# MTG/DeepConvSep

Hardware: NVIDIA H100
Metric: audio_seconds_separated_per_second (higher is better)
Workload: dtype f32

## Files before the change

### deepconvsep_b200/csrc/api.cu

```cuda
#include <stdarg.h>
#include <math.h>
#include <string.h>
#include <stdlib.h>
#include <map>
#include <mutex>
#include <utility>
#include <vector>
#include "common.cuh"

namespace dcs {

static thread_local char g_err[1024] = "";

void set_error(const char* fmt, ...) {
  va_list ap;
  va_start(ap, fmt);
  vsnprintf(g_err, sizeof(g_err), fmt, ap);
  va_end(ap);
}

int DevBuf::ensure(size_t bytes, cudaStream_t stream, bool* grew) {
  if (grew) *grew = false;
  if (bytes <= cap) return DCS_OK;
  if (p) {
// ... 330 lines not shown
}

static bool score_arch(int arch) { return arch == DCS_ARCH_BACH10_SCORE || arch == DCS_ARCH_BACH10_SCORE_1X1; }
static int score_planes(const dcs_model* m) { return m->arch == DCS_ARCH_BACH10_SCORE_1X1 ? 4 : m->sc.nch; }

static int check_model(const char* fn, const dcs_ctx* ctx, const dcs_model* m, int arch, int overlap, int patcher) {
  DCS_REQUIRE(ctx && m, "%s: NULL argument", fn);
  const bool mono = m->arch != DCS_ARCH_DSD_ILD && !score_arch(m->arch);
  DCS_REQUIRE(arch < 0 ? mono : (arch == DCS_ARCH_BACH10_SCORE ? score_arch(m->arch) : m->arch == arch),
              "%s does not serve architecture %d: use %s", fn, m->arch,
              m->arch == DCS_ARCH_DSD_ILD ? "dcs_separate_audio_stereo"
              : score_arch(m->arch)       ? "dcs_separate_audio_score / dcs_separate_spec_channels"
                                          : "dcs_separate_audio / dcs_separate_spec");
  DCS_REQUIRE(overlap >= 0 && overlap < m->tc, "overlap %d must be in [0, time_context=%d)", overlap, m->tc);
  DCS_REQUIRE(patcher == DCS_PATCHER_STANDALONE || patcher == DCS_PATCHER_UTIL, "unknown patcher %d", patcher);
  return DCS_OK;
}

static int check_clip(const char* fn, const dcs_ctx* ctx, const dcs_model* m, const dcs_stft* p, int arch, const void* in,
                      const void* out, int64_t L, int64_t in_stride, int64_t out_stride, int overlap, int patcher) {
  DCS_TRY(check_model(fn, ctx, m, arch, overlap, patcher));
  DCS_REQUIRE(p && in && out, "%s: NULL argument", fn);
  DCS_REQUIRE(p->N / 2 + 1 == m->F, "%s: frame size %d does not give the model's %d bins", fn, p->N, m->F);
  DCS_REQUIRE(L > 0 && in_stride >= L && out_stride >= L, "%s: bad length / stride", fn);
  return DCS_OK;
}

static int size_workspace(dcs_ctx* ctx, const dcs_model* m, const dcs_stft* p, int64_t L, bool staged, cudaStream_t st,
                          bool masks = false) {
  const int64_t plane = dcs_num_frames(L, p->hop) * dcs_padded_bins(p->N);
  if (!masks) DCS_TRY(ctx->X.ensure((size_t)m->nch * plane * sizeof(float2), st));
  DCS_TRY(ctx->mag.ensure((size_t)m->nch * plane * sizeof(float), st));
  if (!masks) DCS_TRY(ctx->S.ensure((size_t)m->nsrc * m->nch * plane * sizeof(float2), st));
  if (score_arch(m->arch)) DCS_TRY(ctx->net[NET_CHANS].ensure((size_t)score_planes(m) * plane * sizeof(float), st));
  if (!masks && ctx->wiener_iters > 0 && m->nch == 2)
    DCS_TRY(ctx->wiener.ensure(wiener_workspace_bytes(m->nsrc, 2, dcs_num_frames(L, p->hop), m->F, ctx->wiener_radius), st));
  if (staged) {
    DCS_TRY(ctx->audio.ensure((size_t)L * sizeof(float), st));
    DCS_TRY(ctx->stems.ensure((size_t)m->nsrc * L * sizeof(float), st));
  }
  return DCS_OK;
}

static int size_downmix_workspace(dcs_ctx* ctx, const dcs_model* m, const dcs_stft* p, int64_t L, int wx, int radius, int staged,
                                  cudaStream_t st) {
  const int64_t plane = dcs_num_frames(L, p->hop) * dcs_padded_bins(p->N);
  DCS_TRY(size_workspace(ctx, m, p, L, false, st, true));
  DCS_TRY(ctx->audio.ensure((size_t)(staged + 1) * L * sizeof(float), st));
  DCS_TRY(ctx->masks.ensure((size_t)m->nsrc * plane * sizeof(float), st));
  DCS_TRY(ctx->X.ensure((size_t)(wx > 0 ? wx : 1) * plane * sizeof(float2), st));
  if (wx > 0) {
    DCS_TRY(ctx->S.ensure((size_t)m->nsrc * wx * plane * sizeof(float2), st));
    DCS_TRY(ctx->wiener.ensure(wiener_workspace_bytes(m->nsrc, wx, dcs_num_frames(L, p->hop), m->F, radius), st));
  }
  if (staged > 0) DCS_TRY(ctx->stems.ensure((size_t)m->nsrc * staged * L * sizeof(float), st));
  return DCS_OK;
}

static int separate_clip(dcs_ctx* ctx, const dcs_model* m, dcs_stft* p, const float* d_audio, int64_t audio_stride, int64_t L,
                         const float* d_filters, const NoteTable* notes, float scale_factor, int overlap, int patcher,
                         float* d_stems, int64_t stem_stride, cudaStream_t st, bool masks = false) {
  DCS_TRY(size_workspace(ctx, m, p, L, false, st, masks));
  const int nch = m->nch;
  const int64_t T = dcs_num_frames(L, p->hop), ldf = dcs_padded_bins(p->N), plane = T * ldf;
  float2 *X = masks ? nullptr : ctx->X.as<float2>(), *S = masks ? nullptr : ctx->S.as<float2>();
  float* mag = ctx->mag.as<float>();
  {
    ProfScope ps(ctx, "stft_fwd", st);
    for (int ch = 0; ch < nch; ++ch)
      DCS_TRY(launch_stft(p, d_audio + ch * audio_stride, L, masks ? nullptr : X + ch * plane, mag + ch * plane, nullptr,
                          scale_factor, ldf, st));
  }
  const float* in = mag;
  if (d_filters || notes) {
    float* chans = ctx->net[NET_CHANS].as<float>();
    ProfScope ps(ctx, "score_channels", st);
    if (notes)
      DCS_TRY(launch_score_notes(ctx, *notes, mag, chans, ldf, plane, st));
    else
      DCS_TRY(launch_channel_mul(ctx, mag, d_filters, chans, plane, score_planes(m), st));
    in = chans;
  }
  if (masks) return run_network(ctx, m, in, plane, nullptr, 0, T, ldf, overlap, patcher, nullptr, stem_stride, st, d_stems);
  DCS_TRY(run_network(ctx, m, in, plane, X, plane, T, ldf, overlap, patcher, S, plane, st));
  if (ctx->wiener_iters > 0 && nch == 2)
    DCS_TRY(launch_wiener(ctx, X, plane, S, plane, m->nsrc, T, ldf, m->F, ctx->wiener_iters, ctx->wiener_radius, st));
  DCS_TRY(copy_tap(ctx, S, (int64_t)m->nsrc * nch * plane, st));
  ProfScope ps(ctx, "istft_ola", st);
  return launch_istft(p, S, nullptr, nullptr, 1.f, m->nsrc * nch, T, ldf, plane, d_stems, L, stem_stride, st);
}

static int apply_masks(dcs_ctx* ctx, dcs_stft* p, const float* d_audio, int nx, int64_t audio_stride, int64_t L,
                       const float* d_masks, int nsrc, int64_t m_stride, float* d_stems, int64_t stem_stride, cudaStream_t st) {
  const int64_t T = dcs_num_frames(L, p->hop), ldf = dcs_padded_bins(p->N), plane = T * ldf;
  DCS_TRY(ctx->X.ensure((size_t)plane * sizeof(float2), st));
  float2* X = ctx->X.as<float2>();
  for (int c = 0; c < nx; ++c) {
    {
      ProfScope ps(ctx, "stft_fwd", st);
      DCS_TRY(launch_stft(p, d_audio + c * audio_stride, L, X, nullptr, nullptr, 1.f, ldf, st));
    }
    ProfScope ps(ctx, "istft_masked", st);
    DCS_TRY(launch_istft(p, X, nullptr, nullptr, 1.f, nsrc, T, ldf, plane, d_stems + c * stem_stride, L, nx * stem_stride, st,
                         d_masks, m_stride, 1));
  }
  return DCS_OK;
}

static int check_keep_tap(const char* fn, const dcs_ctx* ctx) {
  DCS_REQUIRE(!ctx->tap || ctx->wiener_iters > 0,
              "%s: a spectrum tap is set (dcs_set_spectrum_tap), and without the Wiener post-filter this path forms no masked "
              "spectra to copy", fn);
  return DCS_OK;
}

static int downmix_clip(dcs_ctx* ctx, const dcs_model* m, dcs_stft* p, const float* d_mono, const float* d_audio, int nx,
                        int64_t audio_stride, int64_t L, int iterations, int radius, float scale_factor, int overlap,
                        int patcher, float* d_stems, int64_t stem_stride, cudaStream_t st) {
  const bool filter = iterations > 0;
  DCS_TRY(size_downmix_workspace(ctx, m, p, L, filter ? nx : 0, radius, 0, st));
  const int64_t T = dcs_num_frames(L, p->hop), ldf = dcs_padded_bins(p->N), plane = T * ldf;
  float* masks = ctx->masks.as<float>();
  if (!d_mono) {
    ProfScope ps(ctx, "downmix", st);
    DCS_TRY(launch_downmix(ctx, d_audio, nx, audio_stride, L, ctx->audio.as<float>(), st));
    d_mono = ctx->audio.as<float>();
  }
  DCS_TRY(separate_clip(ctx, m, p, d_mono, L, L, nullptr, nullptr, scale_factor, overlap, patcher, masks, plane, st, true));
  if (!filter) return apply_masks(ctx, p, d_audio, nx, audio_stride, L, masks, m->nsrc, plane, d_stems, stem_stride, st);
  float2 *X = ctx->X.as<float2>(), *S = ctx->S.as<float2>();
  {
    ProfScope ps(ctx, "stft_fwd", st);
    for (int c = 0; c < nx; ++c) DCS_TRY(launch_stft(p, d_audio + c * audio_stride, L, X + c * plane, nullptr, nullptr, 1.f, ldf, st));
  }
  DCS_TRY(launch_wiener(ctx, X, plane, S, plane, m->nsrc, T, ldf, m->F, iterations, radius, st, masks, plane, nx));
  DCS_TRY(copy_tap(ctx, S, (int64_t)m->nsrc * nx * plane, st));
  ProfScope ps(ctx, "istft_ola", st);
  return launch_istft(p, S, nullptr, nullptr, 1.f, m->nsrc * nx, T, ldf, plane, d_stems, L, stem_stride, st);
}

int dcs_separate_spec(dcs_ctx* ctx, dcs_model* m, const float* d_mag, const dcs_complex* d_X, int64_t T, int64_t ldf,
                      int overlap, int patcher, dcs_complex* d_S, int64_t src_stride, void* stream) {
  DCS_TRY(check_model("dcs_separate_spec", ctx, m, -1, overlap, patcher));
  DCS_REQUIRE(d_mag && d_X && d_S, "dcs_separate_spec: NULL argument");
  DCS_REQUIRE(T > 0 && ldf >= m->F && src_stride >= T * ldf, "dcs_separate_spec: bad shape");
  DCS_CUDA(cudaSetDevice(ctx->device));
  return run_network(ctx, m, d_mag, 0, (const float2*)d_X, 0, T, ldf, overlap, patcher, (float2*)d_S, src_stride,
                     (cudaStream_t)stream);
}

int dcs_separate_spec_channels(dcs_ctx* ctx, dcs_model* m, const float* d_in, int64_t in_plane, const dcs_complex* d_X,
                               int64_t T, int64_t ldf, int overlap, int patcher, dcs_complex* d_S, int64_t src_stride,
                               void* stream) {
  DCS_TRY(check_model("dcs_separate_spec_channels", ctx, m, DCS_ARCH_BACH10_SCORE, overlap, patcher));
  DCS_REQUIRE(d_in && d_X && d_S, "dcs_separate_spec_channels: NULL argument");
  DCS_REQUIRE(T > 0 && ldf >= m->F && src_stride >= T * ldf && in_plane >= T * ldf, "dcs_separate_spec_channels: bad shape");
  DCS_CUDA(cudaSetDevice(ctx->device));
  return run_network(ctx, m, d_in, in_plane, (const float2*)d_X, 0, T, ldf, overlap, patcher, (float2*)d_S, src_stride,
                     (cudaStream_t)stream);
}

int dcs_separate_audio_score(dcs_ctx* ctx, dcs_model* m, dcs_stft* p, const float* d_audio, int64_t L, const float* d_filters,
                             float scale_factor, int overlap, int patcher, float* d_stems, int64_t stem_stride, void* stream) {
  DCS_TRY(check_clip("dcs_separate_audio_score", ctx, m, p, DCS_ARCH_BACH10_SCORE, d_audio, d_stems, L, L, stem_stride,
                     overlap, patcher));
  DCS_REQUIRE(d_filters, "dcs_separate_audio_score: NULL filters");
// ... 930 lines not shown
```

### deepconvsep_b200/csrc/common.cuh

```cuda
#pragma once
#include <cuda_runtime.h>
#include <stdint.h>
#include <stdio.h>
#include <string>
#include <vector>
#include <string.h>
#include "../../include/dcs.h"

namespace dcs {

void set_error(const char* fmt, ...);

#define DCS_CUDA(expr)                                                                  \
  do {                                                                                  \
    cudaError_t _e = (expr);                                                            \
    if (_e != cudaSuccess) {                                                            \
      dcs::set_error("%s:%d: %s -> %s", __FILE__, __LINE__, #expr, cudaGetErrorString(_e)); \
      return DCS_ECUDA;                                                                 \
    }                                                                                   \
  } while (0)

#define DCS_CHECK_LAUNCH()  DCS_CUDA(cudaGetLastError())

#define DCS_REQUIRE(cond, ...)                 \
// ... 81 lines not shown
struct ProfScope {
  dcs_ctx* c; cudaStream_t st; int idx;
  ProfScope(dcs_ctx* ctx, const char* name, cudaStream_t s) : c(ctx), st(s), idx(-1) {
    if (!c || !c->prof_on) return;
    dcs_prof_rec r; r.name = name;
    if (cudaEventCreate(&r.e0) != cudaSuccess || cudaEventCreate(&r.e1) != cudaSuccess) return;
    cudaEventRecord(r.e0, st);
    c->prof.push_back(r);
    idx = (int)c->prof.size() - 1;
  }
  ~ProfScope() { if (idx >= 0) cudaEventRecord(c->prof[idx].e1, st); }
};
}

namespace dcs {
struct TcWeight {
  float* hi = nullptr;
  float* lo = nullptr;
  int K = 0, N = 0, Kp = 0, Np = 0;
};
}

struct dcs_dsd {
  int C1, C2, kh2, h2, nfc, ndec;
  int C1p, C2p;
  int64_t ldw;
  float *b1, *b2, *bfc, *bdec, *W1t, *bout;
  dcs::TcWeight tW1f, tW2c, tWfc, tWdec, tWt2;
};
struct dcs_sconv {
  int nch, sw1, J, pool, WP, kh2, kw2, h2, w2, HP, WPP, ndec, nfc, rule;
  dcs::TcWeight tW[8];
  float *b1, *b2, *bfc, *bdec[4], *bout, *Wsc;
};
struct dcs_s1x1 {
  int W[7];
  int C[7], CP[7];
  dcs::TcWeight tF[7];
  dcs::TcWeight tI[7];
  float *b[7], *c[7];
  float *bout, *Wsc;
};
struct dcs_model {
  dcs_ctx* ctx;
  int arch, F, tc, nsrc;
  int nch = 1;
  dcs_dsd dsd;
  dcs_sconv sc;
  dcs_s1x1 s1;
  std::vector<void*> dev;
};
namespace dcs {
int upload(const std::vector<float>& h, float** d, std::vector<void*>* owned = nullptr);
int model_create_dsd(dcs_model* m, int nparams, const float* const* hp, const int64_t* shp, const int* nd);
int model_create_sconv(dcs_model* m, int nparams, const float* const* hp, const int64_t* shp, const int* nd);
int model_create_s1x1(dcs_model* m, int nparams, const float* const* hp, const int64_t* shp, const int* nd);
bool shape_is(const int64_t* s, int nd, int want_nd, int64_t a, int64_t b = 1, int64_t c = 1, int64_t d = 1);

struct NetCall {
  const float* in; int64_t in_plane;
  const float2* X; int64_t x_plane;
  float2* S; int64_t src_stride;
  float* M;
  int64_t T, ldf;
  int64_t P, Tp;
  int overlap, step;
  uint64_t sig;
};
int dsd_forward(dcs_ctx* ctx, const dcs_model* m, const NetCall& n, cudaStream_t st);
int sconv_forward(dcs_ctx* ctx, const dcs_model* m, const NetCall& n, cudaStream_t st);
int s1x1_forward(dcs_ctx* ctx, const dcs_model* m, const NetCall& n, cudaStream_t st);
int ensure_layout(dcs_ctx* ctx, NetSlot slot, size_t bytes, uint64_t sig, cudaStream_t st);
}

namespace dcs {

int launch_stft(dcs_stft* plan, const float* d_audio, int64_t L, float2* d_X, float* d_mag,
                float* d_phase, float mag_scale, int64_t ldf, cudaStream_t st);
int launch_istft(dcs_stft* plan, const float2* d_S, const float* d_mag, const float* d_phase,
                 float polar_scale, int nsrc, int64_t T, int64_t ldf, int64_t src_stride, float* d_out,
                 int64_t Lout, int64_t out_stride, cudaStream_t st, const float* d_M = nullptr, int64_t m_stride = 0,
                 int nx = 1);

int launch_stft_reg(dcs_stft* plan, const float* d_audio, int64_t L, float2* d_X, float* d_mag, float* d_phase,
                    float mag_scale, int64_t ldf, int64_t nframes, cudaStream_t st);
bool istft_reg_supported(const dcs_stft* plan, const float* d_out, int64_t out_stride);
int launch_istft_reg(dcs_stft* plan, const float2* d_S, int nsrc, int64_t nframes, int64_t ldf, int64_t src_stride,
                     float* d_out, int64_t Lout, int64_t out_stride, cudaStream_t st, const float* d_M = nullptr,
                     int64_t m_stride = 0, int nx = 1);

struct GemmDesc {
  const float* A; const float* B; const float* bias; float* C;
  int M, N, K;
  int a_valid_rows;
  int m_inner; int64_t a_so, a_si;
  int m_inner2; int64_t a_s2;
  int k_seg; int64_t k_ss;
  int64_t ldb;
  int cm_inner; int64_t c_so, c_si;
  int cm_inner2; int64_t c_s2;
  int n_seg; int64_t n_ss, c_col0;
  int relu;
  int kc_rows, kc_unit, kc_pad, kc_n, kc_taps;
  const float* bias2; uint8_t* code;
  const uint8_t* gate; int g_inner, g_inner2; int64_t g_so, g_si, g_s2, g_lim;
};
enum { EPI_POST = DCS_GEMM_EPI_POST, EPI_GATE = DCS_GEMM_EPI_GATE };
inline bool gemm_c_view_ok(const GemmDesc& d) {
  return d.c_so >= 0 && d.c_si >= 0 && d.c_s2 >= 0 && d.n_ss >= 0 && d.c_col0 >= 0;
}
__host__ __device__ __forceinline__ int64_t gemm_c_row_offset(const GemmDesc& d, int m) {
  return (int64_t)(m / d.cm_inner) * d.c_so + (int64_t)((m % d.cm_inner) / d.cm_inner2) * d.c_si +
         (int64_t)(m % d.cm_inner2) * d.c_s2 + d.c_col0;
}
GemmDesc gemm_plain(const float* A, int64_t lda, const float* B, int64_t ldb, const float* bias, float* C,
                    int64_t ldc, int M, int N, int K, int relu);
int launch_gemm(dcs_ctx* ctx, const GemmDesc& d, cudaStream_t st);

int tc_weight_create(const float* B_rowmajor, int64_t ldb, int K, int N, TcWeight* out, std::vector<void*>* owned = nullptr);
void tc_weight_destroy(TcWeight* w);
int launch_gemm_tc(dcs_ctx* ctx, const GemmDesc& d, const TcWeight& w, cudaStream_t st);
int launch_gemm_tc_epi(dcs_ctx* ctx, const GemmDesc& d, const TcWeight& w, int epi, cudaStream_t st);

struct DsdMaskArgs {
  const float* G;
  int ldg;
  const float* W1t;
  int ldw;
  const float* bout;
  const float2* X;
  float2* S;
  int64_t ldf, src_stride;
  int T, P, tc, overlap, F;
  int ndec;
};
constexpr float MASK_TOT_MIN = 1.2e-38f;
int launch_dsd_mask(dcs_ctx* ctx, const DsdMaskArgs& a, cudaStream_t st, float* M = nullptr);
bool dsd_mask_tc_supported(const DsdMaskArgs& a);
int launch_dsd_mask_tc(dcs_ctx* ctx, const DsdMaskArgs& a, cudaStream_t st, float* M = nullptr);
struct DsdConvT2Args {
  const float* apad;
  float* G;
  int ldg;
  int npairs, tc;
};
bool dsd_convT2_tc_supported(const DsdConvT2Args& a);
int launch_dsd_convT2_tc(dcs_ctx* ctx, const DsdConvT2Args& a, const TcWeight& w, cudaStream_t st);
struct DsdDenseArgs {
  const float* z;
  const float* bias;
  float* apad;
  int P, tc, ndec, nfc;
};
bool dsd_dense_tc_supported(const DsdDenseArgs& a);
int launch_dsd_dense_tc(dcs_ctx* ctx, const DsdDenseArgs& a, const TcWeight& w, cudaStream_t st);
struct SconvMaskArgs {
  int arch;
  const float* G;
  const uint8_t* tie;
  const float* W;
  const float* bout;
  const float2* X;
  float2* S;
  int64_t ldf, src_stride;
  int T, P, tc, overlap, F, J, WP;
  int p_base, t0, t1;
// ... 95 lines not shown
```

### deepconvsep_b200/csrc/stft.cu

```cuda
#include "common.cuh"
#include "fft.cuh"

namespace dcs {

template <int N>
__global__ void __launch_bounds__(N / 8)
stft_kernel(const float* __restrict__ audio, int64_t L, int hop, const float* __restrict__ win,
            const float2* __restrict__ tw, float2* __restrict__ X, float* __restrict__ mag,
            float* __restrict__ phase, int64_t ldf, int64_t T, float mag_scale, int frames_per_cta) {
  constexpr int N2 = N / 2, T4 = N2 / 4, F = N2 + 1;
  __shared__ __align__(16) float2 bufA[N2];
  __shared__ __align__(16) float2 bufB[N2];
  const int tid = threadIdx.x;

  float2 w[4];
#pragma unroll
  for (int m = 0; m < 4; ++m) {
    const int idx = 2 * (tid + m * T4);
    w[m] = make_float2(__ldg(win + idx), __ldg(win + idx + 1));
  }
  const int64_t n0 = (int64_t)blockIdx.x * frames_per_cta;
  for (int f = 0; f < frames_per_cta; ++f) {
    const int64_t n = n0 + f;
    if (n >= T) break;
// ... 315 lines not shown
  const size_t dyn = (size_t)span * sizeof(float);
  if (d_M) {
    dim3 grid((unsigned)(ceil_div64(Lout, span) * nsrc), (unsigned)nx);
    DCS_TRY(ensure_smem_attr(istft_masked_kernel<N>, 96 * 1024));
    istft_masked_kernel<N><<<grid, N / 8, dyn, st>>>(d_S, T, ldf, src_stride, d_M, m_stride, nsrc, nx, p->d_wsyn, p->d_w2,
                                                     p->d_tw, d_out, Lout, out_stride, p->hop, hpc);
    DCS_CHECK_LAUNCH();
    p->ctx->launches++;
    return DCS_OK;
  }
  dim3 grid((unsigned)ceil_div64(Lout, span), (unsigned)nsrc);
  DCS_TRY(ensure_smem_attr(istft_kernel<N>, 96 * 1024));
  istft_kernel<N><<<grid, N / 8, dyn, st>>>(d_S, d_mag, d_phase, polar_scale, T, ldf, src_stride, p->d_wsyn, p->d_w2,
                                            p->d_tw, d_out, Lout, out_stride, p->hop, hpc);
  DCS_CHECK_LAUNCH();
  p->ctx->launches++;
  return DCS_OK;
}

int launch_istft(dcs_stft* p, const float2* d_S, const float* d_mag, const float* d_phase, float polar_scale,
                 int nsrc, int64_t T, int64_t ldf, int64_t src_stride, float* d_out, int64_t Lout,
                 int64_t out_stride, cudaStream_t st, const float* d_M, int64_t m_stride, int nx) {
  DCS_REQUIRE(Lout <= (T - 1) * p->hop + p->N - p->N / 2, "num_out %lld exceeds the istft length", (long long)Lout);
  if (Lout <= 0 || nsrc <= 0 || nx <= 0) return DCS_OK;
  const bool mask_rows_ok = !d_M || (ldf % 4 == 0 && m_stride % 4 == 0 && (uintptr_t)d_M % 16 == 0 && ldf >= p->N / 2 + 4);
  if (d_S && istft_reg_supported(p, d_out, out_stride) && ldf % 2 == 0 &&
      src_stride % 2 == 0 && ((uintptr_t)d_S % 16 == 0) && ldf >= (p->N / 2 + 2) / 2 * 2 && mask_rows_ok)
    return launch_istft_reg(p, d_S, nsrc, T, ldf, src_stride, d_out, Lout, out_stride, st, d_M, m_stride, nx);
#define DCS_ISTFT_CASE(NN) \
  case NN: return launch_istft_n<NN>(p, d_S, d_mag, d_phase, polar_scale, nsrc, T, ldf, src_stride, d_out, Lout, out_stride, st, d_M, m_stride, nx);
  switch (p->N) {
    DCS_ISTFT_CASE(256)
    DCS_ISTFT_CASE(512)
    DCS_ISTFT_CASE(1024)
    DCS_ISTFT_CASE(2048)
    DCS_ISTFT_CASE(4096)
  }
#undef DCS_ISTFT_CASE
  DCS_REQUIRE(false, "unsupported frame size %d", p->N);
}

int launch_pcm_decode(dcs_ctx* ctx, const int16_t* d_pcm, int64_t L, int channels, int downmix, float* d_audio,
                      cudaStream_t st) {
  if (L <= 0) return DCS_OK;
  pcm_decode_kernel<<<(unsigned)ceil_div64(L, 256), 256, 0, st>>>(d_pcm, L, channels, downmix, d_audio);
  DCS_CHECK_LAUNCH();
  ctx->launches++;
  return DCS_OK;
}

template <int FMT>
static void pcm_decode_channels_as(const void* d_in, int64_t L, int C, float* d_planes, cudaStream_t st) {
  pcm_decode_channels_kernel<FMT><<<(unsigned)ceil_div64(L, 256), 256, 0, st>>>(
      static_cast<const typename SampleFormat<FMT>::T*>(d_in), L, C, d_planes);
}

template <int FMT>
static void pcm_encode_channels_as(const float* d_stems, int64_t L, int nsrc, int C, int64_t stem_stride, void* d_out,
                                   cudaStream_t st) {
  dim3 grid((unsigned)ceil_div64(L, kPcmEncodeRows), (unsigned)nsrc);
  pcm_encode_channels_kernel<FMT><<<grid, kPcmEncodeRows, 0, st>>>(d_stems, L, C, stem_stride,
                                                                   static_cast<typename SampleFormat<FMT>::T*>(d_out));
}

int launch_pcm_decode_channels(dcs_ctx* ctx, int fmt, const void* d_in, int64_t L, int C, float* d_planes, cudaStream_t st) {
  if (L <= 0) return DCS_OK;
  DCS_REQUIRE(C >= 1 && C <= kPcmMaxChannels, "pcm_decode_channels: %d channels not in [1, %d]", C, kPcmMaxChannels);
  DCS_REQUIRE(sample_bytes(fmt) > 0 && (uintptr_t)d_in % sample_align(fmt) == 0,
              "pcm_decode_channels: format %d, or input not aligned to its samples", fmt);
  switch (fmt) {
    case DCS_SAMPLE_I16: pcm_decode_channels_as<DCS_SAMPLE_I16>(d_in, L, C, d_planes, st); break;
    case DCS_SAMPLE_I32: pcm_decode_channels_as<DCS_SAMPLE_I32>(d_in, L, C, d_planes, st); break;
    case DCS_SAMPLE_I24:
      pcm24_decode_channels_kernel<<<(unsigned)ceil_div64(L, kPcmEncodeRows), kPcmEncodeRows, 0, st>>>(
          static_cast<const uint8_t*>(d_in), L, C, d_planes);
      break;
    default: pcm_decode_channels_as<DCS_SAMPLE_F32>(d_in, L, C, d_planes, st); break;
  }
  DCS_CHECK_LAUNCH();
  ctx->launches++;
  return DCS_OK;
}

int launch_downmix(dcs_ctx* ctx, const float* d_audio, int nx, int64_t audio_stride, int64_t L, float* d_mono, cudaStream_t st) {
  if (L <= 0) return DCS_OK;
  downmix_kernel<<<(unsigned)ceil_div64(L, 256), 256, 0, st>>>(d_audio, nx, audio_stride, L, d_mono);
  DCS_CHECK_LAUNCH();
  ctx->launches++;
  return DCS_OK;
}

int launch_pcm_encode_channels(dcs_ctx* ctx, int fmt, const float* d_stems, int64_t L, int nsrc, int C, int64_t stem_stride,
                               void* d_out, cudaStream_t st) {
  if (L <= 0) return DCS_OK;
  DCS_REQUIRE(C >= 1 && C <= kPcmMaxChannels, "pcm_encode_channels: %d channels not in [1, %d]", C, kPcmMaxChannels);
  DCS_REQUIRE(sample_bytes(fmt) > 0 && (uintptr_t)d_out % sample_align(fmt) == 0,
              "pcm_encode_channels: format %d, or output not aligned to its samples", fmt);
  switch (fmt) {
    case DCS_SAMPLE_I16: pcm_encode_channels_as<DCS_SAMPLE_I16>(d_stems, L, nsrc, C, stem_stride, d_out, st); break;
    case DCS_SAMPLE_I32: pcm_encode_channels_as<DCS_SAMPLE_I32>(d_stems, L, nsrc, C, stem_stride, d_out, st); break;
    case DCS_SAMPLE_I24:
      pcm24_encode_channels_kernel<<<dim3((unsigned)ceil_div64(L, kPcmEncodeRows), (unsigned)nsrc), kPcmEncodeRows, 0, st>>>(
          d_stems, L, C, stem_stride, static_cast<uint8_t*>(d_out));
      break;
    default: pcm_encode_channels_as<DCS_SAMPLE_F32>(d_stems, L, nsrc, C, stem_stride, d_out, st); break;
  }
  DCS_CHECK_LAUNCH();
  ctx->launches++;
  return DCS_OK;
}

int launch_pcm_encode(dcs_ctx* ctx, const float* d_stems, int64_t L, int nsrc, int64_t stem_stride, int16_t* d_out,
                      int64_t out_stride, cudaStream_t st) {
  if (L <= 0) return DCS_OK;
  dim3 grid((unsigned)ceil_div64(L, 256), (unsigned)nsrc);
  pcm_encode_kernel<<<grid, 256, 0, st>>>(d_stems, L, stem_stride, d_out, out_stride);
  DCS_CHECK_LAUNCH();
  ctx->launches++;
  return DCS_OK;
}

}
```

### deepconvsep_b200/csrc/stft_reg.cu

```cuda
#include "common.cuh"
#include "fft_reg.cuh"

namespace dcs {

constexpr int REG_THREADS = 128;
constexpr int ISTFT_THREADS = 256;

template <int T>
__global__ void __launch_bounds__(REG_THREADS)
stft_reg_kernel(const float* __restrict__ audio, int64_t L, int hop, const float* __restrict__ win,
                const float2* __restrict__ tw, float2* __restrict__ X, float* __restrict__ mag,
                float* __restrict__ phase, int64_t ldf, int64_t nframes, float mag_scale, int frames_per_group) {
  using G = FftGroup<T>;
  constexpr int N2 = G::N2, N = 2 * N2, F = N2 + 1, GPC = REG_THREADS / T;
  extern __shared__ __align__(16) float2 scratch[];
  const int tid = threadIdx.x, b = tid % T, gl = tid / T;
  float2* scr = scratch + gl * G::SCRATCH;
  float2* stw = scratch + GPC * G::SCRATCH;
  float2* stw2 = stw + N2;
  float2* swin = stw2 + N2;
  for (int i = tid; i < N2; i += REG_THREADS) stw[i] = __ldg(tw + i);
  G::fill_tw2(stw2, tw, tid, REG_THREADS);
  for (int i = tid; i < N2; i += REG_THREADS) swin[i] = __ldg(reinterpret_cast<const float2*>(win) + i);
  __syncthreads();
  const int64_t g = (int64_t)blockIdx.x * GPC + gl;
  const bool audio_aligned8 = (reinterpret_cast<uintptr_t>(audio) & 7) == 0;
  const int64_t warp_first = ((int64_t)blockIdx.x * GPC + (tid / 32) * (32 / T)) * frames_per_group;
  for (int i = 0; i < frames_per_group; ++i) {
    if (warp_first + i >= nframes) break;
    const int64_t n = g * frames_per_group + i;
    const bool valid = n < nframes;
    const int64_t base = n * hop - N / 2;
    float2 v[32];
    if (valid && base >= 0 && base + N <= L && audio_aligned8) {
      const float2* __restrict__ ap = reinterpret_cast<const float2*>(audio + base);
#pragma unroll
      for (int a = 0; a < 32; ++a) {
        const int idx = a * T + b;
        const float2 w = swin[idx], x = __ldg(ap + idx);
        v[a] = make_float2(x.x * w.x, x.y * w.y);
      }
    } else {
#pragma unroll
      for (int a = 0; a < 32; ++a) {
        const int idx = a * T + b;
        const int64_t s = base + 2 * idx;
        const float2 w = swin[idx];
        const float x0 = (valid && s >= 0 && s < L) ? __ldg(audio + s) : 0.f;
        const float x1 = (valid && s + 1 >= 0 && s + 1 < L) ? __ldg(audio + s + 1) : 0.f;
        v[a] = make_float2(x0 * w.x, x1 * w.y);
      }
    }
    G::template forward<true>(v, scr, stw2, b);
#pragma unroll
    for (int q = 0; q < G::Q; ++q)
#pragma unroll
      for (int kb = 0; kb < T; ++kb) scr[(b + T * q) + 32 * kb] = v[q * T + kb];
    __syncwarp();
    if (valid) {
      const int64_t row = n * ldf;
#pragma unroll 4
      for (int m = 0; m < N2 / T; ++m) {
        const int k = b + T * m;
        const float2 xk = real_post_shared<N2>(scr, stw, k);
        if (X) X[row + k] = xk;
        if (mag) mag[row + k] = mag_scale * sqrtf(xk.x * xk.x + xk.y * xk.y);
        if (phase) phase[row + k] = atan2f(xk.y, xk.x);
      }
      if (b == 0) {
        const float2 z0 = scr[0];
        const float vv = z0.x - z0.y;
        if (X) X[row + N2] = make_float2(vv, 0.f);
        if (mag) mag[row + N2] = mag_scale * fabsf(vv);
        if (phase) phase[row + N2] = atan2f(0.f, vv);
      }
      if (b < ldf - F) {
        if (X) X[row + F + b] = make_float2(0.f, 0.f);
        if (mag) mag[row + F + b] = 0.f;
        if (phase) phase[row + F + b] = 0.f;
      }
    }
    __syncwarp();
  }
}

template <int T, int HS, bool MASKED>
__device__ __forceinline__ void
istft_reg_body(const float2* __restrict__ S, int64_t nframes, int64_t ldf, int64_t src_stride,
               const float* __restrict__ wsyn, const float* __restrict__ w2, const float2* __restrict__ tw,
               float* __restrict__ out, int64_t Lout, int64_t out_stride, int hops_per_group, int64_t num_hops,
               int64_t groups_per_src, int64_t total_groups, const float* __restrict__ Mk, int64_t m_stride, int nsrc,
               int nx) {
  using G = FftGroup<T>;
  constexpr int N2 = G::N2, N = 2 * N2, hop = 64 * HS, R = N / hop, C0 = (N / 2) / hop, GPC = ISTFT_THREADS / T;
  extern __shared__ __align__(16) float2 scratch[];
  const int tid = threadIdx.x, b = tid % T, gl = tid / T;
  float2* scr = scratch + gl * G::SCRATCH;
  int64_t gi = (int64_t)blockIdx.x * GPC + gl;
  const bool active = gi < total_groups;
  if (!active) gi = total_groups - 1;
  int msrc = 0;
  if constexpr (MASKED) {
    msrc = (int)(gi % nsrc);
    gi /= nsrc;
  }
  const int src = (int)(gi / groups_per_src);
  const int64_t h0 = (gi % groups_per_src) * hops_per_group;
  const float inv_n2 = 1.0f / (float)N2;
  float2 acc[32];
#pragma unroll
  for (int i = 0; i < 32; ++i) acc[i] = make_float2(0.f, 0.f);
  float* o = out + (int64_t)(MASKED ? msrc * nx + src : src) * out_stride;
  float2 cinv[G::Q * HS];
#pragma unroll
  for (int q = 0; q < G::Q; ++q)
#pragma unroll
    for (int kb = 0; kb < HS; ++kb) {
      const int e = 2 * ((b + T * q) + 32 * kb);
      float c0 = 0.f, c1 = 0.f;
#pragma unroll
      for (int r = 0; r < R; ++r) {
        const float2 ww = __ldg(reinterpret_cast<const float2*>(w2 + e + r * hop));
        c0 += ww.x;
        c1 += ww.y;
      }
      cinv[q * HS + kb] = make_float2(c0 == 0.f ? 1.f : 1.f / c0, c1 == 0.f ? 1.f : 1.f / c1);
    }

  constexpr int ROWP = (N2 + 1 + 7) / 8 * 8;
  constexpr int CHUNKS = (N2 + 2) / 2;
  float2* srow = scratch + GPC * G::SCRATCH + gl * ROWP;
  float2* stw = scratch + GPC * (G::SCRATCH + ROWP);
  float2* stw2 = stw + N2;
  float2* swsyn = stw2 + N2;
  constexpr int MCHUNKS = (N2 + 4) / 4;
  float* smrow = reinterpret_cast<float*>(swsyn + N2) + gl * ROWP;
  for (int i = tid; i < N2; i += ISTFT_THREADS) stw[i] = __ldg(tw + i);
  G::fill_tw2(stw2, tw, tid, ISTFT_THREADS);
  for (int i = tid; i < N2; i += ISTFT_THREADS) swsyn[i] = __ldg(reinterpret_cast<const float2*>(wsyn) + i);
  __syncthreads();
  auto prefetch = [&](int64_t nn) {
    if (nn >= 0 && nn < nframes) {
      const float2* rowp = S + (int64_t)src * src_stride + nn * ldf;
      for (int c = b; c < CHUNKS; c += T) {
        const uint32_t dst = (uint32_t)__cvta_generic_to_shared(srow + 2 * c);
        asm volatile("cp.async.cg.shared.global [%0], [%1], 16;" ::"r"(dst), "l"(rowp + 2 * c) : "memory");
      }
      if constexpr (MASKED) {
        const float* mrowp = Mk + (int64_t)msrc * m_stride + nn * ldf;
        for (int c = b; c < MCHUNKS; c += T) {
          const uint32_t dst = (uint32_t)__cvta_generic_to_shared(smrow + 4 * c);
          asm volatile("cp.async.cg.shared.global [%0], [%1], 16;" ::"r"(dst), "l"(mrowp + 4 * c) : "memory");
        }
      }
    }
    asm volatile("cp.async.commit_group;" ::: "memory");
  };
  const int64_t n_first = h0 + C0 - R + 1, n_last = h0 + hops_per_group - 1 + C0;
  prefetch(n_first);
  for (int64_t n = n_first; n <= n_last; ++n) {
    const bool fvalid = n >= 0 && n < nframes;
    asm volatile("cp.async.wait_group 0;" ::: "memory");
    __syncwarp();
    float2 v[32];
#pragma unroll
    for (int a = 0; a < 32; ++a) {
      const int idx = a * T + b;
      float2 xk = make_float2(0.f, 0.f), xn = xk;
      if (fvalid) {
        xk = srow[idx];
        xn = srow[N2 - idx];
        if constexpr (MASKED) {
          const float mk = smrow[idx], mn = smrow[N2 - idx];
          xk = make_float2(__fmul_rn(mk, xk.x), __fmul_rn(mk, xk.y));
          xn = make_float2(__fmul_rn(mn, xn.x), __fmul_rn(mn, xn.y));
        }
      }
      if (idx == 0) { xk.y = 0.f; xn.y = 0.f; }
      v[a] = real_pre_conj(xk, xn, stw[idx]);
    }
    __syncwarp();
    if (n < n_last) prefetch(n + 1);
    G::template forward<true>(v, scr, stw2, b);
#pragma unroll
    for (int q = 0; q < G::Q; ++q)
#pragma unroll
      for (int kb = 0; kb < T; ++kb) {
        const int np = (b + T * q) + 32 * kb;
        const float2 w = swsyn[np];
        const float2 r = v[q * T + kb];
        acc[q * T + kb].x = fmaf(w.x, r.x * inv_n2, acc[q * T + kb].x);
        acc[q * T + kb].y = fmaf(w.y, -r.y * inv_n2, acc[q * T + kb].y);
      }
    const int64_t h = n - C0;
    if (active && h >= h0 && h < num_hops) {
      const bool interior = (n - (R - 1) >= 0) && (n < nframes);
#pragma unroll
      for (int q = 0; q < G::Q; ++q)
#pragma unroll
        for (int kb = 0; kb < HS; ++kb) {
          const int e = 2 * ((b + T * q) + 32 * kb);
          float2 ic = cinv[q * HS + kb];
          if (!interior) {
            float c0 = 0.f, c1 = 0.f;
#pragma unroll
            for (int r = 0; r < R; ++r) {
              const int64_t nf = n - r;
              if (nf >= 0 && nf < nframes) {
                const float2 ww = __ldg(reinterpret_cast<const float2*>(w2 + e + r * hop));
                c0 += ww.x;
                c1 += ww.y;
              }
            }
            ic = make_float2(c0 == 0.f ? 1.f : 1.f / c0, c1 == 0.f ? 1.f : 1.f / c1);
          }
          const int64_t oi = h * hop + e;
          const float2 a2 = acc[q * T + kb];
          if (oi + 1 < Lout) {
            *reinterpret_cast<float2*>(o + oi) = make_float2(a2.x * ic.x, a2.y * ic.y);
          } else if (oi < Lout) {
            o[oi] = a2.x * ic.x;
          }
        }
    }
#pragma unroll
    for (int q = 0; q < G::Q; ++q) {
#pragma unroll
      for (int kb = 0; kb < T - HS; ++kb) acc[q * T + kb] = acc[q * T + kb + HS];
#pragma unroll
      for (int kb = T - HS; kb < T; ++kb) acc[q * T + kb] = make_float2(0.f, 0.f);
    }
  }
}

template <int T, int HS>
__global__ void __launch_bounds__(ISTFT_THREADS, 1)
istft_reg_kernel(const float2* __restrict__ S, int64_t nframes, int64_t ldf, int64_t src_stride,
                 const float* __restrict__ wsyn, const float* __restrict__ w2, const float2* __restrict__ tw,
                 float* __restrict__ out, int64_t Lout, int64_t out_stride, int hops_per_group, int64_t num_hops,
                 int64_t groups_per_src, int64_t total_groups) {
  istft_reg_body<T, HS, false>(S, nframes, ldf, src_stride, wsyn, w2, tw, out, Lout, out_stride, hops_per_group, num_hops,
                               groups_per_src, total_groups, nullptr, 0, 1, 1);
}

template <int T, int HS>
__global__ void __launch_bounds__(ISTFT_THREADS, 1)
istft_masked_reg_kernel(const float2* __restrict__ X, int64_t nframes, int64_t ldf, int64_t x_plane,
                        const float* __restrict__ Mk, int64_t m_stride, int nsrc, int nx, const float* __restrict__ wsyn,
                        const float* __restrict__ w2, const float2* __restrict__ tw, float* __restrict__ out, int64_t Lout,
                        int64_t out_stride, int hops_per_group, int64_t num_hops, int64_t groups_per_plane,
                        int64_t total_groups) {
  istft_reg_body<T, HS, true>(X, nframes, ldf, x_plane, wsyn, w2, tw, out, Lout, out_stride, hops_per_group, num_hops,
                              groups_per_plane, total_groups, Mk, m_stride, nsrc, nx);
}

int launch_stft_reg(dcs_stft* p, const float* d_audio, int64_t L, float2* d_X, float* d_mag, float* d_phase,
                    float mag_scale, int64_t ldf, int64_t nframes, cudaStream_t st) {
  const int fpg = 4;
  const float ms = mag_scale / sqrtf((float)p->N);
  if (p->N == 2048) {
    using G = FftGroup<32>;
    const int gpc = REG_THREADS / 32;
    const size_t smem = (gpc * G::SCRATCH + 3 * G::N2) * sizeof(float2);
    DCS_TRY(ensure_smem_attr(stft_reg_kernel<32>, (int)smem));
    const unsigned grid = (unsigned)ceil_div64(nframes, (int64_t)gpc * fpg);
    stft_reg_kernel<32><<<grid, REG_THREADS, smem, st>>>(
        d_audio, L, p->hop, p->d_win, p->d_tw, d_X, d_mag, d_phase, ldf, nframes, ms, fpg);
  } else {
    using G = FftGroup<16>;
    const int gpc = REG_THREADS / 16;
    const size_t smem = (gpc * G::SCRATCH + 3 * G::N2) * sizeof(float2);
    DCS_TRY(ensure_smem_attr(stft_reg_kernel<16>, (int)smem));
    const unsigned grid = (unsigned)ceil_div64(nframes, (int64_t)gpc * fpg);
    stft_reg_kernel<16><<<grid, REG_THREADS, smem, st>>>(
        d_audio, L, p->hop, p->d_win, p->d_tw, d_X, d_mag, d_phase, ldf, nframes, ms, fpg);
  }
  DCS_CHECK_LAUNCH();
  p->ctx->launches++;
  return DCS_OK;
}

bool istft_reg_supported(const dcs_stft* p, const float* d_out, int64_t out_stride) {
  return (p->N == 1024 || p->N == 2048) && (p->hop == 512 || p->hop == 256) && ((uintptr_t)d_out % 8 == 0) &&
         out_stride % 2 == 0;
}

template <int T, int HS>
static int launch_istft_reg_t(dcs_stft* p, const float2* d_S, int nsrc, int64_t nframes, int64_t ldf, int64_t src_stride,
                              float* d_out, int64_t Lout, int64_t out_stride, cudaStream_t st, const float* d_M = nullptr,
                              int64_t m_stride = 0, int nx = 1) {
  using G = FftGroup<T>;
  constexpr int GPC = ISTFT_THREADS / T;
  const int hop = 64 * HS;
  const int64_t num_hops = ceil_div64(Lout, hop);
  const int64_t target_groups = (int64_t)p->ctx->num_sms * (ISTFT_THREADS / 32) * (32 / T);
  const int nplanes = nsrc * nx;
  int64_t hpg = ceil_div64((int64_t)nplanes * num_hops, target_groups);
  if (hpg < 12) hpg = 12;
  if (hpg > 64) hpg = 64;
  const int64_t groups_per_src = ceil_div64(num_hops, hpg);
  const int64_t total = groups_per_src * nplanes;
  const unsigned grid = (unsigned)ceil_div64(total, GPC);
  constexpr int ROWP = (G::N2 + 1 + 7) / 8 * 8;
  const size_t smem = ((size_t)GPC * (G::SCRATCH + ROWP) + 2 * G::N2 + G::N2) * sizeof(float2);
  if (d_M) {
    const size_t smem_m = smem + (size_t)GPC * ROWP * sizeof(float);
    DCS_TRY(ensure_smem_attr(istft_masked_reg_kernel<T, HS>, (int)smem_m));
    istft_masked_reg_kernel<T, HS><<<grid, ISTFT_THREADS, smem_m, st>>>(
        d_S, nframes, ldf, src_stride, d_M, m_stride, nsrc, nx, p->d_wsyn, p->d_w2, p->d_tw, d_out, Lout, out_stride,
        (int)hpg, num_hops, groups_per_src, total);
  } else {
    DCS_TRY(ensure_smem_attr(istft_reg_kernel<T, HS>, (int)smem));
    istft_reg_kernel<T, HS><<<grid, ISTFT_THREADS, smem, st>>>(
        d_S, nframes, ldf, src_stride, p->d_wsyn, p->d_w2, p->d_tw, d_out, Lout, out_stride, (int)hpg, num_hops,
        groups_per_src, total);
  }
  DCS_CHECK_LAUNCH();
  p->ctx->launches++;
  return DCS_OK;
}

int launch_istft_reg(dcs_stft* p, const float2* d_S, int nsrc, int64_t nframes, int64_t ldf, int64_t src_stride,
                     float* d_out, int64_t Lout, int64_t out_stride, cudaStream_t st, const float* d_M, int64_t m_stride,
                     int nx) {
#define DCS_ISTFT_REG_CASE(NN, HOP) \
  if (p->N == NN && p->hop == HOP)  \
    return launch_istft_reg_t<NN / 64, HOP / 64>(p, d_S, nsrc, nframes, ldf, src_stride, d_out, Lout, out_stride, st, d_M, m_stride, nx);
  DCS_ISTFT_REG_CASE(2048, 512)
  DCS_ISTFT_REG_CASE(2048, 256)
  DCS_ISTFT_REG_CASE(1024, 512)
  DCS_ISTFT_REG_CASE(1024, 256)
#undef DCS_ISTFT_REG_CASE
  DCS_REQUIRE(false, "istft_reg: unsupported frame size / hop");
}

}
```

Before: 152,600.

## Fuse mask application into masked iSTFT with TMA bulk-copy ring and shared mixture rows

For mono DSD models, the network now writes masks instead of masked spectra, and the iSTFT applies them on the fly from the shared mixture spectrum. This skips materialising per-source complex spectra, and a separate kernel builds them only when a tap is requested. The iSTFT row prefetch moves from per-thread cp.async to mbarrier-synchronised bulk copies with a two-slot ring. In the masked path, groups working on different sources for the same hop range share one mixture row load. This cuts global traffic and load instructions, but adds mbarrier synchronisation complexity and larger shared-memory use, which can limit occupancy.

```diff
diff --git a/deepconvsep_b200/csrc/api.cu b/deepconvsep_b200/csrc/api.cu
--- a/deepconvsep_b200/csrc/api.cu
+++ b/deepconvsep_b200/csrc/api.cu
@@ -436,6 +436,17 @@
     in = chans;
   }
   if (masks) return run_network(ctx, m, in, plane, nullptr, 0, T, ldf, overlap, patcher, nullptr, stem_stride, st, d_stems);
+  if (m->arch == DCS_ARCH_DSD && nch == 1 && istft_reg_supported(p, d_stems, stem_stride)) {
+    float* M = reinterpret_cast<float*>(S);
+    DCS_TRY(run_network(ctx, m, in, plane, X, plane, T, ldf, overlap, patcher, nullptr, plane, st, M));
+    if (ctx->tap) {
+      DCS_REQUIRE(ctx->tap_cap >= (int64_t)m->nsrc * plane, "spectrum tap holds %lld elements, this call produced %lld",
+                  (long long)ctx->tap_cap, (long long)m->nsrc * plane);
+      DCS_TRY(launch_masked_spectra(ctx, M, X, m->nsrc, plane, ldf, m->F, ctx->tap, st));
+    }
+    ProfScope ps(ctx, "istft_ola", st);
+    return launch_istft(p, X, nullptr, nullptr, 1.f, m->nsrc, T, ldf, plane, d_stems, L, stem_stride, st, M, plane, 1);
+  }
   DCS_TRY(run_network(ctx, m, in, plane, X, plane, T, ldf, overlap, patcher, S, plane, st));
   if (ctx->wiener_iters > 0 && nch == 2)
     DCS_TRY(launch_wiener(ctx, X, plane, S, plane, m->nsrc, T, ldf, m->F, ctx->wiener_iters, ctx->wiener_radius, st));
diff --git a/deepconvsep_b200/csrc/common.cuh b/deepconvsep_b200/csrc/common.cuh
--- a/deepconvsep_b200/csrc/common.cuh
+++ b/deepconvsep_b200/csrc/common.cuh
@@ -187,6 +187,9 @@
                  int64_t Lout, int64_t out_stride, cudaStream_t st, const float* d_M = nullptr, int64_t m_stride = 0,
                  int nx = 1);
 
+int launch_masked_spectra(dcs_ctx* ctx, const float* d_M, const float2* d_X, int nsrc, int64_t plane, int64_t ldf, int F,
+                          float2* d_S, cudaStream_t st);
+
 int launch_stft_reg(dcs_stft* plan, const float* d_audio, int64_t L, float2* d_X, float* d_mag, float* d_phase,
                     float mag_scale, int64_t ldf, int64_t nframes, cudaStream_t st);
 bool istft_reg_supported(const dcs_stft* plan, const float* d_out, int64_t out_stride);
diff --git a/deepconvsep_b200/csrc/stft.cu b/deepconvsep_b200/csrc/stft.cu
--- a/deepconvsep_b200/csrc/stft.cu
+++ b/deepconvsep_b200/csrc/stft.cu
@@ -421,6 +421,30 @@
   return DCS_OK;
 }
 
+__global__ void masked_spectra_kernel(const float* __restrict__ M, const float2* __restrict__ X, int64_t plane, int64_t ldf, int F,
+                                      int64_t n, float2* __restrict__ S) {
+  const int64_t i = (int64_t)blockIdx.x * blockDim.x + threadIdx.x;
+  if (i >= n) return;
+  const int64_t e = i % plane, f = e % ldf;
+  if (f < F) {
+    const float m = M[i];
+    const float2 x = X[e];
+    S[i] = make_float2(__fmul_rn(m, x.x), __fmul_rn(m, x.y));
+  } else {
+    S[i] = make_float2(0.f, 0.f);
+  }
+}
+
+int launch_masked_spectra(dcs_ctx* ctx, const float* d_M, const float2* d_X, int nsrc, int64_t plane, int64_t ldf, int F,
+                          float2* d_S, cudaStream_t st) {
+  const int64_t n = (int64_t)nsrc * plane;
+  if (n <= 0) return DCS_OK;
+  masked_spectra_kernel<<<(unsigned)ceil_div64(n, 256), 256, 0, st>>>(d_M, d_X, plane, ldf, F, n, d_S);
+  DCS_CHECK_LAUNCH();
+  ctx->launches++;
+  return DCS_OK;
+}
+
 int launch_downmix(dcs_ctx* ctx, const float* d_audio, int nx, int64_t audio_stride, int64_t L, float* d_mono, cudaStream_t st) {
   if (L <= 0) return DCS_OK;
   downmix_kernel<<<(unsigned)ceil_div64(L, 256), 256, 0, st>>>(d_audio, nx, audio_stride, L, d_mono);
diff --git a/deepconvsep_b200/csrc/stft_reg.cu b/deepconvsep_b200/csrc/stft_reg.cu
--- a/deepconvsep_b200/csrc/stft_reg.cu
+++ b/deepconvsep_b200/csrc/stft_reg.cu
@@ -1,5 +1,6 @@
 #include "common.cuh"
 #include "fft_reg.cuh"
+#include "tc.cuh"
 
 namespace dcs {
 
@@ -84,28 +85,47 @@
   }
 }
 
+constexpr int ISTFT_RING = 2;
+constexpr size_t SM90_SMEM_OPTIN = 232448;
+template <int T>
+__host__ __device__ constexpr int istft_rowp() { return (32 * T + 1 + 7) / 8 * 8; }
+template <int T>
+__host__ __device__ constexpr size_t istft_smem_bytes(int qpc, bool masked) {
+  constexpr int GPC = ISTFT_THREADS / T, ROWP = istft_rowp<T>();
+  return ((size_t)GPC * FftGroup<T>::SCRATCH + 3 * (size_t)(32 * T) + (size_t)qpc * ISTFT_RING * ROWP) * sizeof(float2) +
+         (masked ? (size_t)GPC * ISTFT_RING * ROWP * sizeof(float) : 0) +
+         ((size_t)qpc * 2 * ISTFT_RING + (masked ? (size_t)GPC * ISTFT_RING : 0)) * sizeof(uint64_t);
+}
+
 template <int T, int HS, bool MASKED>
 __device__ __forceinline__ void
 istft_reg_body(const float2* __restrict__ S, int64_t nframes, int64_t ldf, int64_t src_stride,
                const float* __restrict__ wsyn, const float* __restrict__ w2, const float2* __restrict__ tw,
                float* __restrict__ out, int64_t Lout, int64_t out_stride, int hops_per_group, int64_t num_hops,
-               int64_t groups_per_src, int64_t total_groups, const float* __restrict__ Mk, int64_t m_stride, int nsrc,
-               int nx) {
+               int64_t groups_per_src, int64_t total_quads, const float* __restrict__ Mk, int64_t m_stride, int nsrc,
+               int nx, int qw, int qpc) {
   using G = FftGroup<T>;
   constexpr int N2 = G::N2, N = 2 * N2, hop = 64 * HS, R = N / hop, C0 = (N / 2) / hop, GPC = ISTFT_THREADS / T;
+  constexpr int ROWP = istft_rowp<T>();
+  constexpr uint32_t XBYTES = (N2 + 2) / 2 * 16;
+  constexpr uint32_t MBYTES = (N2 + 4) / 4 * 16;
   extern __shared__ __align__(16) float2 scratch[];
   const int tid = threadIdx.x, b = tid % T, gl = tid / T;
   float2* scr = scratch + gl * G::SCRATCH;
-  int64_t gi = (int64_t)blockIdx.x * GPC + gl;
-  const bool active = gi < total_groups;
-  if (!active) gi = total_groups - 1;
+  const int qi = gl / qw, mem = gl - qi * qw;
+  const bool in_quad = qi < qpc;
+  int64_t gq = (int64_t)blockIdx.x * qpc + (in_quad ? qi : 0);
+  bool active = in_quad && gq < total_quads;
+  if (gq >= total_quads) gq = total_quads - 1;
   int msrc = 0;
   if constexpr (MASKED) {
-    msrc = (int)(gi % nsrc);
-    gi /= nsrc;
-  }
-  const int src = (int)(gi / groups_per_src);
-  const int64_t h0 = (gi % groups_per_src) * hops_per_group;
+    const int nchunk = (nsrc + qw - 1) / qw;
+    msrc = (int)(gq % nchunk) * qw + mem;
+    gq /= nchunk;
+    if (msrc >= nsrc) { active = false; msrc = nsrc - 1; }
+  }
+  const int src = (int)(gq / groups_per_src);
+  const int64_t h0 = (gq % groups_per_src) * hops_per_group;
   const float inv_n2 = 1.0f / (float)N2;
   float2 acc[32];
 #pragma unroll
@@ -127,41 +147,65 @@
       cinv[q * HS + kb] = make_float2(c0 == 0.f ? 1.f : 1.f / c0, c1 == 0.f ? 1.f : 1.f / c1);
     }
 
-  constexpr int ROWP = (N2 + 1 + 7) / 8 * 8;
-  constexpr int CHUNKS = (N2 + 2) / 2;
-  float2* srow = scratch + GPC * G::SCRATCH + gl * ROWP;
-  float2* stw = scratch + GPC * (G::SCRATCH + ROWP);
+  float2* stw = scratch + GPC * G::SCRATCH;
   float2* stw2 = stw + N2;
   float2* swsyn = stw2 + N2;
-  constexpr int MCHUNKS = (N2 + 4) / 4;
-  float* smrow = reinterpret_cast<float*>(swsyn + N2) + gl * ROWP;
+  float2* xring = swsyn + N2 + (in_quad ? qi : 0) * ISTFT_RING * ROWP;
+  float* mring = reinterpret_cast<float*>(swsyn + N2 + qpc * ISTFT_RING * ROWP) + gl * ISTFT_RING * ROWP;
+  uint64_t* bars = reinterpret_cast<uint64_t*>(reinterpret_cast<float*>(swsyn + N2 + qpc * ISTFT_RING * ROWP) +
+                                               (MASKED ? GPC * ISTFT_RING * ROWP : 0));
+  uint64_t* xfull = bars + (in_quad ? qi : 0) * 2 * ISTFT_RING;
+  uint64_t* xempty = xfull + ISTFT_RING;
+  uint64_t* mfull = bars + qpc * 2 * ISTFT_RING + gl * ISTFT_RING;
   for (int i = tid; i < N2; i += ISTFT_THREADS) stw[i] = __ldg(tw + i);
   G::fill_tw2(stw2, tw, tid, ISTFT_THREADS);
   for (int i = tid; i < N2; i += ISTFT_THREADS) swsyn[i] = __ldg(reinterpret_cast<const float2*>(wsyn) + i);
+  if (tid < qpc * ISTFT_RING) {
+    tc::mbar_init(bars + (tid / ISTFT_RING) * 2 * ISTFT_RING + tid % ISTFT_RING, 1);
+    tc::mbar_init(bars + (tid / ISTFT_RING) * 2 * ISTFT_RING + ISTFT_RING + tid % ISTFT_RING, (uint32_t)qw);
+  }
+  if (MASKED && tid < GPC * ISTFT_RING) tc::mbar_init(bars + qpc * 2 * ISTFT_RING + tid, 1);
+  tc::fence_barrier_init();
   __syncthreads();
-  auto prefetch = [&](int64_t nn) {
+  const bool xlane = in_quad && mem == 0 && b == 0;
+  const bool glane = in_quad && b == 0;
+  const int64_t n_first = h0 + C0 - R + 1, n_last = h0 + hops_per_group - 1 + C0;
+  auto fetch_x = [&](int64_t nn) {
+    const int k = (int)(nn - n_first), st = k % ISTFT_RING;
+    if (k >= ISTFT_RING)
+      tc::mbar_wait_relaxed(xempty + st, (uint32_t)((k / ISTFT_RING - 1) & 1));
     if (nn >= 0 && nn < nframes) {
-      const float2* rowp = S + (int64_t)src * src_stride + nn * ldf;
-      for (int c = b; c < CHUNKS; c += T) {
-        const uint32_t dst = (uint32_t)__cvta_generic_to_shared(srow + 2 * c);
-        asm volatile("cp.async.cg.shared.global [%0], [%1], 16;" ::"r"(dst), "l"(rowp + 2 * c) : "memory");
-      }
-      if constexpr (MASKED) {
-        const float* mrowp = Mk + (int64_t)msrc * m_stride + nn * ldf;
-        for (int c = b; c < MCHUNKS; c += T) {
-          const uint32_t dst = (uint32_t)__cvta_generic_to_shared(smrow + 4 * c);
-          asm volatile("cp.async.cg.shared.global [%0], [%1], 16;" ::"r"(dst), "l"(mrowp + 4 * c) : "memory");
-        }
-      }
-    }
-    asm volatile("cp.async.commit_group;" ::: "memory");
+      tc::mbar_arrive_expect_tx(xfull + st, XBYTES);
+      tc::bulk_copy_g2s(xring + st * ROWP, S + (int64_t)src * src_stride + nn * ldf, XBYTES, xfull + st);
+    } else {
+      tc::mbar_arrive(xfull + st);
+    }
   };
-  const int64_t n_first = h0 + C0 - R + 1, n_last = h0 + hops_per_group - 1 + C0;
-  prefetch(n_first);
+  auto fetch_m = [&](int64_t nn) {
+    const int st = (int)(nn - n_first) % ISTFT_RING;
+    if (nn >= 0 && nn < nframes) {
+      tc::mbar_arrive_expect_tx(mfull + st, MBYTES);
+      tc::bulk_copy_g2s(mring + st * ROWP, Mk + (int64_t)msrc * m_stride + nn * ldf, MBYTES, mfull + st);
+    } else {
+      tc::mbar_arrive(mfull + st);
+    }
+  };
+  if (xlane) fetch_x(n_first);
+  if (MASKED && glane) fetch_m(n_first);
   for (int64_t n = n_first; n <= n_last; ++n) {
-    const bool fvalid = n >= 0 && n < nframes;
-    asm volatile("cp.async.wait_group 0;" ::: "memory");
-    __syncwarp();
+    const bool fvalid = in_quad && n >= 0 && n < nframes;
+    const int k = (int)(n - n_first), st = k % ISTFT_RING;
+    const uint32_t par = (uint32_t)((k / ISTFT_RING) & 1);
+    if (n < n_last) {
+      if (xlane) fetch_x(n + 1);
+      if (MASKED && glane) fetch_m(n + 1);
+    }
+    const float2* srow = xring + st * ROWP;
+    const float* smrow = mring + st * ROWP;
+    if (in_quad) {
+      tc::mbar_wait(xfull + st, par);
+      if constexpr (MASKED) tc::mbar_wait(mfull + st, par);
+    }
     float2 v[32];
 #pragma unroll
     for (int a = 0; a < 32; ++a) {
@@ -180,7 +224,7 @@
       v[a] = real_pre_conj(xk, xn, stw[idx]);
     }
     __syncwarp();
-    if (n < n_last) prefetch(n + 1);
+    if (glane) tc::mbar_arrive(xempty + st);
     G::template forward<true>(v, scr, stw2, b);
 #pragma unroll
     for (int q = 0; q < G::Q; ++q)
@@ -240,7 +284,7 @@
                  float* __restrict__ out, int64_t Lout, int64_t out_stride, int hops_per_group, int64_t num_hops,
                  int64_t groups_per_src, int64_t total_groups) {
   istft_reg_body<T, HS, false>(S, nframes, ldf, src_stride, wsyn, w2, tw, out, Lout, out_stride, hops_per_group, num_hops,
-                               groups_per_src, total_groups, nullptr, 0, 1, 1);
+                               groups_per_src, total_groups, nullptr, 0, 1, 1, 1, ISTFT_THREADS / T);
 }
 
 template <int T, int HS>
@@ -249,9 +293,9 @@
                         const float* __restrict__ Mk, int64_t m_stride, int nsrc, int nx, const float* __restrict__ wsyn,
                         const float* __restrict__ w2, const float2* __restrict__ tw, float* __restrict__ out, int64_t Lout,
                         int64_t out_stride, int hops_per_group, int64_t num_hops, int64_t groups_per_plane,
-                        int64_t total_groups) {
+                        int64_t total_quads, int qw, int qpc) {
   istft_reg_body<T, HS, true>(X, nframes, ldf, x_plane, wsyn, w2, tw, out, Lout, out_stride, hops_per_group, num_hops,
-                              groups_per_plane, total_groups, Mk, m_stride, nsrc, nx);
+                              groups_per_plane, total_quads, Mk, m_stride, nsrc, nx, qw, qpc);
 }
 
 int launch_stft_reg(dcs_stft* p, const float* d_audio, int64_t L, float2* d_X, float* d_mag, float* d_phase,
@@ -289,7 +333,6 @@
 static int launch_istft_reg_t(dcs_stft* p, const float2* d_S, int nsrc, int64_t nframes, int64_t ldf, int64_t src_stride,
                               float* d_out, int64_t Lout, int64_t out_stride, cudaStream_t st, const float* d_M = nullptr,
                               int64_t m_stride = 0, int nx = 1) {
-  using G = FftGroup<T>;
   constexpr int GPC = ISTFT_THREADS / T;
   const int hop = 64 * HS;
   const int64_t num_hops = ceil_div64(Lout, hop);
@@ -299,17 +342,21 @@
   if (hpg < 12) hpg = 12;
   if (hpg > 64) hpg = 64;
   const int64_t groups_per_src = ceil_div64(num_hops, hpg);
-  const int64_t total = groups_per_src * nplanes;
-  const unsigned grid = (unsigned)ceil_div64(total, GPC);
-  constexpr int ROWP = (G::N2 + 1 + 7) / 8 * 8;
-  const size_t smem = ((size_t)GPC * (G::SCRATCH + ROWP) + 2 * G::N2 + G::N2) * sizeof(float2);
   if (d_M) {
-    const size_t smem_m = smem + (size_t)GPC * ROWP * sizeof(float);
-    DCS_TRY(ensure_smem_attr(istft_masked_reg_kernel<T, HS>, (int)smem_m));
-    istft_masked_reg_kernel<T, HS><<<grid, ISTFT_THREADS, smem_m, st>>>(
+    const int qw = nsrc < GPC ? nsrc : GPC;
+    int qpc = GPC / qw;
+    while (qpc > 1 && istft_smem_bytes<T>(qpc, true) > SM90_SMEM_OPTIN) --qpc;
+    const int64_t quads = groups_per_src * nx * ((nsrc + qw - 1) / qw);
+    const unsigned grid = (unsigned)ceil_div64(quads, qpc);
+    const size_t smem = istft_smem_bytes<T>(qpc, true);
+    DCS_TRY(ensure_smem_attr(istft_masked_reg_kernel<T, HS>, (int)smem));
+    istft_masked_reg_kernel<T, HS><<<grid, ISTFT_THREADS, smem, st>>>(
         d_S, nframes, ldf, src_stride, d_M, m_stride, nsrc, nx, p->d_wsyn, p->d_w2, p->d_tw, d_out, Lout, out_stride,
-        (int)hpg, num_hops, groups_per_src, total);
+        (int)hpg, num_hops, groups_per_src, quads, qw, qpc);
   } else {
+    const int64_t total = groups_per_src * nplanes;
+    const unsigned grid = (unsigned)ceil_div64(total, GPC);
+    const size_t smem = istft_smem_bytes<T>(GPC, false);
     DCS_TRY(ensure_smem_attr(istft_reg_kernel<T, HS>, (int)smem));
     istft_reg_kernel<T, HS><<<grid, ISTFT_THREADS, smem, st>>>(
         d_S, nframes, ldf, src_stride, p->d_wsyn, p->d_w2, p->d_tw, d_out, Lout, out_stride, (int)hpg, num_hops,
```

Result: faster. 162,600, median of 6 (+6.5%).
